# Griffan/FASTQuick

Measured on AMD Instinct MI355X. Metric: paired_150bp_reads_aligned_per_sec, higher is better.
Workload: dtype u32

## Files before the change

fastquick_amd/api.py:

```python
from __future__ import annotations

import ctypes as C
import os

import numpy as np

HERE = os.path.dirname(os.path.abspath(__file__))
DEFAULT_LIB = os.environ.get("FQ_LIB_EXPERIMENT") or os.path.join(HERE, "libfastquick_amd.so")

FQ_K_NAMES = ("prep", "width", "gap", "sa", "sw", "refine", "prep_kernel", "gap_kernel")


class Opts(C.Structure):
    _fields_ = [
        ("s_mm", C.c_int32), ("s_gapo", C.c_int32), ("s_gape", C.c_int32), ("mode", C.c_int32),
        ("indel_end_skip", C.c_int32), ("max_del_occ", C.c_int32), ("max_entries", C.c_int32),
        ("fnr", C.c_double), ("max_diff", C.c_int32), ("max_gapo", C.c_int32), ("max_gape", C.c_int32),
        ("max_seed_diff", C.c_int32), ("seed_len", C.c_int32), ("max_top2", C.c_int32), ("trim_qual", C.c_int32),
        ("filter_thresh", C.c_int32), ("max_isize", C.c_int32), ("force_isize", C.c_int32), ("max_occ", C.c_uint32),
        ("n_multi", C.c_int32), ("N_multi", C.c_int32), ("is_sw", C.c_int32), ("ap_prior", C.c_double),
        ("host_threads", C.c_int32), ("batch_pairs", C.c_int32), ("single_end", C.c_int32), ("pad_opts", C.c_int32),
    ]


# ... 35 lines not shown
class Isize(C.Structure):
    _fields_ = [("avg", C.c_double), ("std", C.c_double), ("ap_prior", C.c_double), ("low", C.c_uint32),
                ("high", C.c_uint32), ("high_bayesian", C.c_uint32), ("pad", C.c_uint32)]


class ResultBatch(C.Structure):
    _fields_ = [("n_pairs", C.c_int32), ("n_survivors", C.c_int32), ("n_both_filtered", C.c_int32),
                ("n_both_unmapped", C.c_int32), ("pair_idx", C.POINTER(C.c_int32)), ("rec", C.POINTER(Result)),
                ("cigar", C.POINTER(C.c_uint16)), ("md", C.c_void_p), ("multi", C.POINTER(Multi)),
                ("isize", Isize), ("n_bases", C.c_int64), ("n_sub", C.c_int32), ("isize_sub", C.POINTER(Isize))]


class Stats(C.Structure):
    _fields_ = [("kernel_ms", C.c_double * 16), ("kernel_launches", C.c_uint64 * 16),
                ("occ_block_touches", C.c_uint64), ("gap_occ_touches", C.c_uint64), ("gap_nogap_touches", C.c_uint64), ("filter_probes", C.c_uint64),
                ("stack_pops", C.c_uint64), ("stack_pushes", C.c_uint64), ("sa_rows", C.c_uint64),
                ("reads_searched", C.c_uint64), ("pairs", C.c_uint64), ("sw_tasks", C.c_uint64),
                ("refine_tasks", C.c_uint64), ("tier_retries", C.c_uint64),
                ("max_pops_per_read", C.c_uint64), ("reads_over_4k_pops", C.c_uint64), ("max_wave_trips", C.c_uint64),
                ("host_ms_serial", C.c_double), ("host_ms_pair", C.c_double), ("host_ms_total", C.c_double),
                ("wall_ms_total", C.c_double), ("wave_trips", C.c_uint64), ("lane_trips", C.c_uint64),
                ("h2d_bytes", C.c_uint64), ("d2h_bytes", C.c_uint64), ("pairs_on_device", C.c_uint64), ("dbg", C.c_uint64 * 16),
                ("width_occ_touches", C.c_uint64), ("md_reads", C.c_uint64), ("host_pairs", C.c_uint64),
                ("device_wait_ms", C.c_double), ("host_cpu_ms", C.c_double), ("dp_launches", C.c_uint64 * 6)]


class FrontEndStats(C.Structure):
    _fields_ = [("ms_inflate", C.c_double), ("ms_tokenise", C.c_double), ("members", C.c_int64), ("refused", C.c_int64),
                ("text_bytes", C.c_int64), ("comp_bytes", C.c_int64), ("pairs", C.c_int64),
                ("ms_lines", C.c_double), ("ms_records", C.c_double), ("ms_slots", C.c_double), ("inflate_launches", C.c_int64), ("chunks", C.c_int64),
                ("ms_wait_reader", C.c_double), ("ms_wait_slot", C.c_double), ("ms_read", C.c_double), ("ms_upload", C.c_double),
                ("bam_records", C.c_int64), ("bam_skipped", C.c_int64), ("chain_repairs", C.c_int64), ("ms_transcode", C.c_double),
                ("ms_bam_starts", C.c_double), ("ms_bam_pairs", C.c_double), ("ms_bam_fill", C.c_double),
                ("bam_orphans", C.c_int64), ("bam_held_peak_records", C.c_int64), ("bam_held_peak_bytes", C.c_int64), ("ms_bam_collate", C.c_double),
                ("bam_unselected", C.c_int64), ("bam_oq_records", C.c_int64), ("ms_bam_tags", C.c_double), ("bam_empty_chunks", C.c_int64)]


class BamCollate(C.Structure):
    _fields_ = [("records", C.c_int64), ("kept", C.c_int64), ("pairs", C.c_int64), ("orphans", C.c_int64), ("held_peak_records", C.c_int64), ("held_peak_bytes", C.c_int64),
                ("text_len", C.c_int64 * 2), ("chain_end", C.c_int64), ("bad_record", C.c_int64),
                ("bad_kind", C.c_int32), ("paired", C.c_int32), ("chunks", C.c_int32), ("end_flag", C.c_int32),
                ("ms_collate", C.c_double), ("ms_keys", C.c_double), ("ms_sort", C.c_double), ("ms_match", C.c_double), ("ms_units", C.c_double), ("ms_hold", C.c_double),
                ("error", C.c_char * 256)]


class BamProbe(C.Structure):
    _fields_ = [("n_ref", C.c_int32), ("paired", C.c_int32), ("first_flag", C.c_int32), ("first_l_seq", C.c_int32), ("first_l_name", C.c_int32), ("has_eof_block", C.c_int32),
# ... 1189 lines not shown
```

fastquick_amd/csrc/fq_align.cpp:

```cpp
#include <algorithm>
#include <atomic>
#include <ctime>
#include <chrono>
#include <climits>
#include <cstdint>
#include <cmath>
#include <cstdio>
#include <cstdlib>
#include <cstring>
#include <memory>
#include <string>
#include <unordered_map>
#include <mutex>
#include <thread>
#include <vector>
#include <pthread.h>
#include <sched.h>

#include "../../include/fastquick_amd.h"
#include "fq_backend.h"
#include "fq_index.h"
#include "fq_pipeline.h"
#include "fq_pool.h"
#include "fq_text_batch.h"
// ... 381 lines not shown
  else if (k == "gap_split_hard") c->kn.gap_split_hard = v;
  else if (k == "gap_long_pops2") c->kn.gap_long_pops2 = (uint32_t)v;
  else if (k == "gap_skip_bound") c->kn.gap_skip_bound = v;
  else if (k == "gap_no_order") c->kn.gap_no_order = (int)v;
  else if (k == "device_turns") c->kn.device_turns = (int)v;
  else if (k == "device_turn_min") c->kn.device_turn_min = v;
  else if (k == "device_turn_slots") c->kn.device_turn_slots = (int)std::max<int64_t>(1, v);
  else if (k == "gap_round2_waves") c->kn.gap_round2_waves = (int)v;
  else if (k == "gap_round2_lane_major") c->kn.gap_round2_lane_major = (int)v;
  else if (k == "gap_round1_refill") c->kn.gap_round1_refill = (int)v;
  else if (k == "gap_round2_refill") c->kn.gap_round2_refill = (int)v;
  else if (k == "sw_wave_max") c->kn.sw_wave_max = (int)v;
  else if (k == "host_threads") c->kn.host_threads = (int)v;
  else if (k == "host_par_min") c->kn.host_par_min = (size_t)v;
  else if (k == "packed_bulk_min") c->kn.packed_bulk_min = v;
  else if (k == "md_mask_min") c->kn.md_mask_min = v;
  else if (k == "trace") c->kn.trace = (int)v;
  else if (k == "gap_order_asc") t->gap_order_asc = (int)v;
  else if (k == "gap_waves_per_cu") t->gap_waves_per_cu = (int)v;
  else if (k == "gap_coop_waves") t->gap_coop_waves = (int)v;
  else if (k == "gap_refill_min") t->gap_refill_min = (int)v;
  else if (k == "filter_no_turns") t->filter_no_turns = (int)v;
  else if (k == "prep_priority") t->prep_priority = (int)v;
  else if (k == "refine_lanes") t->refine_lanes = (int)v;
  else if (k == "gap_generic_opts") t->gap_generic_opts = (int)v;
  else if (k == "sw_serial_reverse") t->sw_serial_reverse = (int)v;
  else if (k == "width_both_strands") t->width_both_strands = (int)v;
  else if (k == "spin_sync") t->spin_sync = (int)v;
  else return FQ_EINVAL;
  return FQ_OK;
}

extern "C" void fq_stats_get(const fq_ctx_t *c, fq_stats_t *out) { if (c && out) *out = c->stats; }
extern "C" void fq_stats_reset(fq_ctx_t *c) { if (c) memset(&c->stats, 0, sizeof c->stats); }

#define CK(expr)                                                  \
  do {                                                            \
    if ((expr)) { c->err = std::string(#expr) + ": " + fqdev::last_error(); return FQ_ENODEV; } \
  } while (0)
#define CKM(expr)                                                 \
  do {                                                            \
    if (!(expr)) { c->err = std::string("out of device memory: ") + #expr; return FQ_ENOMEM; } \
  } while (0)

static int h2d_staged(fq_ctx *c, void *dst, const void *src, size_t bytes) {
  if (!bytes) return 0;
// ... 303 lines not shown
  const fq_text_batch *text = nullptr;
};

int stage0_filter(Call &K, const FilterIn &in) {
  fq_ctx *c = K.c;
  const int n = K.n, n2 = K.n2, n_sub = K.n_sub, B = K.B;
  const bool ascii = !in.head, se = c->o.single_end != 0, ragged = !ascii && in.uniform_len <= 0;
  const int n_in = se ? n : n2;
  const size_t n_max = (size_t)(ascii ? 1 : 3) * n_sub;
  CKM(c->d_filtered.ensure(n2 + 64) && c->d_read_list.ensure(n2) && c->d_sidx.ensure(n2) && c->d_pair_list.ensure(n) && c->d_sub_max.ensure(n_max) && (!ascii || c->d_len_trim.ensure(n2)));
  CK(fqdev::dzero(c->d_sub_max.p, n_max * 4));
  if (se) CK(fqdev::dfill(c->d_filtered.p + n, 1, (size_t)n));
  if (se && ascii) CK(fqdev::dzero(c->d_len_trim.p + n, (size_t)n * 4));
  fqdev::time_begin(FQ_K_PREP);
  if (ascii) {
    FqPrepArgs a{};
    a.ix = c->ix->dev; a.o = c->ko; a.seq = c->d_seq.p; a.qual = c->d_qual.p; a.len = c->d_len.p; a.stride = c->stride; a.n_reads = n_in;
    a.len_trim = c->d_len_trim.p; a.filtered = c->d_filtered.p; a.sub_max = c->d_sub_max.p; a.n_pairs = n; a.batch_pairs = B; a.counters = c->d_counters.p;
    CK(fqdev::launch_prep(a));
  } else {
    FqPrepPackedArgs a{};
    a.ix = c->ix->dev; a.o = c->ko; a.head = in.head; a.len = ragged ? in.len : nullptr; a.uniform_len = in.uniform_len; a.qual_last = in.qual_last; a.sub_whole = c->d_sub_max.p + n_sub;
    a.n_reads = n_in; a.filtered = c->d_filtered.p; a.sub_max = c->d_sub_max.p; a.n_pairs = n; a.batch_pairs = B; a.counters = c->d_counters.p;
    CK(fqdev::launch_prep_packed(a));
  }
  CK(fqdev::launch_compact(c->d_filtered.p, n, c->d_read_list.p, c->d_sidx.p, c->d_pair_list.p, c->d_counts.p));
  fqdev::time_end(FQ_K_PREP);
  int32_t counts[2] = {0, 0};
  c->h_sub_max.assign(n_sub, in.uniform_len);
  K.sub_whole.assign(n_sub, 0);
  std::vector<uint64_t> striped(ragged ? (size_t)FQ_C_STRIPES * FQ_C_STRIDE : 0);
  CKS(d2h_staged(c, counts, c->d_counts.p, 8));
  if (in.qual_last) CKS(d2h_staged(c, K.sub_whole.data(), c->d_sub_max.p + n_sub, (size_t)n_sub * 4));
  if (ascii || ragged) CKS(d2h_staged(c, c->h_sub_max.data(), c->d_sub_max.p, (size_t)n_sub * 4));
  if (ragged) CKS(d2h_staged(c, striped.data(), c->d_counters.p, striped.size() * 8));
  CKS(sync_staged(c));
  K.trace("  stage0: filter + compaction on the device");
  if (ragged) {
    uint64_t folded[FQ_C_COUNT];
    fold_counters(striped.data(), folded);
    if (folded[FQ_C_BADLEN]) return refuse_length(c);
    for (int sb = 0; in.body_stride && sb < n_sub; ++sb)
      if (((int64_t)c->h_sub_max[sb] + 3) / 4 > (int64_t)in.body_stride) { c->err = "a read is longer than body_stride holds"; return FQ_EINVAL; }
    c->n_bases_in = (int64_t)folded[FQ_C_BASES];
  } else if (!ascii) c->n_bases_in = (int64_t)n_in * in.uniform_len;
  K.n_search = counts[0]; K.n_surv = counts[1];
  K.dstride = ascii ? c->stride : (std::max(1, *std::max_element(c->h_sub_max.begin(), c->h_sub_max.end())) + 15) & ~15;
// ... 1780 lines not shown
```

fastquick_amd/csrc/fq_backend.h:

```cpp
#pragma once
#include "fq_kernels.h"
#include "fq_records.h"
#include "fq_frontend.h"
#include "fq_emit.h"
#include "fq_deflate.h"
#include "fq_sort.h"
#include "fq_bamin.h"

namespace fqdev {

struct State;
struct Tune {
  int gap_coop_waves = 0;
  int gap_waves_per_cu = 0, gap_refill_min = 0, gap_order_asc = 0, filter_no_turns = 0, refine_lanes = 0;
  int spin_sync = 0;
  int gap_generic_opts = 0;
  int width_both_strands = 0;
  int prep_priority = 0;
  int sw_serial_reverse = 0;
};
int runtime_configure(int hw_queues, int blocking_waits);
int device_count();
State *state_create(int device_ordinal);
void state_destroy(State *s);
int bind(State *s);
Tune *tune(State *s);
const char *last_error();
bool is_real_gpu();
void device_turn_begin(int slots = 1);
void device_turn_end();

void *dmalloc(size_t bytes);
void dfree(void *p);
void *hmalloc(size_t bytes);
void hfree(void *p);
int h2d(void *dst, const void *src, size_t bytes);
int d2h(void *dst, const void *src, size_t bytes);
int copy_pinned(void *dst, const void *src, size_t bytes, int to_device);
int d2d(void *dst, const void *src, size_t bytes);
int dzero(void *dst, size_t bytes);
int dfill(void *dst, int byte, size_t bytes);
int sync();
int h2d_copy(void *dst, const void *src, size_t bytes);
int copy_record(int slot);
int copy_wait(int slot);
void copy_discard();
int compute_wait_copy(int slot);
int copy_flush_now();

void time_begin(int kid);
void time_end(int kid);
void time_collect(double ms[], uint64_t launches[], int n_ids);
inline thread_local uint64_t dp_launches[FQ_DP_COUNT] = {};

int launch_prep(const FqPrepArgs &a);
int launch_compact(const uint8_t *filtered, int n_pairs, int32_t *read_list, int32_t *sidx, int32_t *pair_list, int32_t *counts);
int launch_surv_gather(const int32_t *pair_list, int n_surv, int n_pairs, const int32_t *len_trim, const uint8_t *filtered, const int32_t *sidx, FqSurvInfo *out);
int launch_prep_packed(const FqPrepPackedArgs &a);
int launch_surv_map(const int32_t *pair_list, int n_surv, int n_pairs, const uint8_t *filtered, const int32_t *sidx, FqSurvInfo *out,
                    int32_t *row_map, int32_t *read_list_c, int32_t *crow_of);
int launch_unpack(const FqUnpackArgs &a);
int launch_patch(const FqPatchArgs &a);
int launch_trim(const FqTrimArgs &a);
int launch_trim_all(const FqTrimAllArgs &a);
int launch_width(const FqWidthArgs &a);
int launch_order(const uint8_t *bid_end, int n, int n_hard, int32_t *order, uint32_t *cnt);
int gap_lane_slots(const FqGapArgs &a);
int launch_gap(const FqGapArgs &a);
int launch_scan(const uint32_t *in, uint64_t *out, uint32_t n);
int launch_pack_aln(const FqAln *aln, const uint32_t *n_aln, const uint64_t *off, uint32_t cap, uint32_t n_work, FqAln *packed);
int launch_sa(const FqSaArgs &a);
int stream_aux(int on);
int stream_fork();
int stream_join();
int stream_mark(int k);
int stream_wait_mark(int k);
// ... 27 lines not shown
```

fastquick_amd/csrc/fq_device.hip:

```cpp
#include <hip/hip_runtime.h>
#include <hip/hip_ext.h>

#include <algorithm>
#include <condition_variable>
#include <atomic>
#include <cstdio>
#include <cstdlib>
#include <cstring>
#include <mutex>
#include <string>
#include <unordered_map>
#include <vector>
#include <sys/mman.h>
#include <sys/syscall.h>
#include <unistd.h>

#include "fq_backend.h"
#define FQ_PC_KERNELS
#include "fq_popcon.h"
#define FQ_SVD_KERNELS
#include "fq_svd.h"
#define FQ_VCF_KERNELS
#include "fq_vcf.h"

// ... 33 lines not shown
      return -3;                                                                             \
    }                                                                                        \
  } while (0)

int copy_flush();
#define FQ_PRE() do { if (copy_flush()) return -3; } while (0)
void copy_discard() { if (g_cur) g_cur->n_small = 0; }
int copy_flush_now() { FQ_PRE(); return 0; }

const char *last_error() { return g_err.c_str(); }
bool is_real_gpu() { return true; }

static int set_kernel_attributes();
static std::mutex g_dev_mu;
static bool g_dev_ready[64];
static hipEvent_t g_prep_last[64];
static State *g_prep_owner[64];
static hipStream_t g_copy_streams[64][2];
static unsigned g_copy_next[64];
static std::mutex g_turn_mu[64];
static std::condition_variable g_turn_cv[64];
static int g_turn_held[64];
static int g_ctx_count[64];
static hipStream_t g_prio_stream[64];
static bool g_queue_warned = false;
static int g_rt_blocking_waits = 0;
int runtime_configure(int hw_queues, int blocking_waits) {
  if (hw_queues > 0) {
    char b[16];
    snprintf(b, sizeof b, "%d", hw_queues);
    setenv("GPU_MAX_HW_QUEUES", b, 0);
  }
  g_rt_blocking_waits = blocking_waits ? 1 : 0;
  return 0;
}

int device_count() { int n = 0; if (hipGetDeviceCount(&n) != hipSuccess) { (void)hipGetLastError(); return 0; } return n < 0 ? 0 : n; }
void device_turn_begin(int slots) {
  const int d = g_cur->device;
  std::unique_lock<std::mutex> lk(g_turn_mu[d]);
  g_turn_cv[d].wait(lk, [&] { return g_turn_held[d] < (slots < 1 ? 1 : slots); });
  ++g_turn_held[d];
}
void device_turn_end() {
  const int d = g_cur->device;
  { std::lock_guard<std::mutex> lk(g_turn_mu[d]); --g_turn_held[d]; }
// ... 28 lines not shown
            hipEventCreateWithFlags(&s->copy_done[1], hipEventDisableTiming | hipEventBlockingSync) == hipSuccess &&
            hipEventCreateWithFlags(&s->prep_done, hipEventDisableTiming) == hipSuccess &&
            hipEventCreateWithFlags(&s->sync_ev, hipEventDisableTiming | hipEventBlockingSync) == hipSuccess;
  if (!ok) { g_err = "stream / event creation failed"; state_destroy(s); return nullptr; }
  s->main_stream = s->stream;
  return s;
}
void state_destroy(State *s) {
  if (!s) return;
  (void)hipSetDevice(s->device);
  g_cur = nullptr;
  s->stream = s->main_stream ? s->main_stream : s->stream;
  if (s->aux_stream) { (void)hipStreamSynchronize(s->aux_stream); (void)hipStreamDestroy(s->aux_stream); }
  if (s->sync_ev) (void)hipEventDestroy(s->sync_ev);
  if (s->fork_ev) (void)hipEventDestroy(s->fork_ev);
  if (s->join_ev) (void)hipEventDestroy(s->join_ev);
  for (hipEvent_t m : s->marks) if (m) (void)hipEventDestroy(m);
  if (s->prio_fork) (void)hipEventDestroy(s->prio_fork);
  if (s->stream) (void)hipStreamSynchronize(s->stream);
  if (s->copy_stream) (void)hipStreamSynchronize(s->copy_stream);
  {
    std::lock_guard<std::mutex> lk(g_dev_mu);
    if (g_prep_owner[s->device] == s) { g_prep_owner[s->device] = nullptr; g_prep_last[s->device] = nullptr; }
    if (g_ctx_count[s->device] > 0) --g_ctx_count[s->device];
  }
  for (auto &p : s->pending) { (void)hipEventDestroy(p.a); (void)hipEventDestroy(p.b); }
  for (auto e : s->free_events) (void)hipEventDestroy(e);
  for (auto e : s->copy_done) if (e) (void)hipEventDestroy(e);
  if (s->prep_done) (void)hipEventDestroy(s->prep_done);
  if (s->scan_tmp) (void)hipFree(s->scan_tmp);
  if (s->cmp_cnt) (void)hipFree(s->cmp_cnt);
  if (s->cmp_off) (void)hipFree(s->cmp_off);
  if (s->stream) (void)hipStreamDestroy(s->stream);
  delete s;
}
Tune *tune(State *s) { return &s->tune; }
int bind(State *s) {
  if (!s) { g_err = "no device state"; return -3; }
  if (g_cur != s) { FQ_HIP(hipSetDevice(s->device)); g_cur = s; }
  return 0;
}

void *dmalloc(size_t bytes) {
  void *p = nullptr;
  if (hipMalloc(&p, bytes ? bytes : 16) != hipSuccess) { g_err = "hipMalloc failed (" + std::to_string(bytes) + " B)"; return nullptr; }
  return p;
}
// ... 889 lines not shown
    FQ_HIP(hipEventRecord(g_cur->prep_done, g_stream));
    g_prep_last[dev] = g_cur->prep_done; g_prep_owner[dev] = g_cur;
  } else {
    hipExtLaunchKernelGGL(k_prep, dim3(nblk((uint64_t)a.n_reads, 256)), dim3(256), 0, g_stream, e0, e1, 0, a);
  }
  FQ_HIP(hipGetLastError());
  return 0;
}
__global__ void __launch_bounds__(256) k_surv_gather(const int32_t *pair_list, int n_surv, int n_pairs, const int32_t *len_trim, const uint8_t *filtered, const int32_t *sidx, FqSurvInfo *out) {
  const int t = blockIdx.x * blockDim.x + threadIdx.x;
  if (t < 2 * n_surv) fq_surv_gather_thread(pair_list, n_pairs, len_trim, filtered, sidx, out, t);
}
int launch_surv_gather(const int32_t *pair_list, int n_surv, int n_pairs, const int32_t *len_trim, const uint8_t *filtered, const int32_t *sidx, FqSurvInfo *out) {
  FQ_PRE();
  if (n_surv <= 0) return 0;
  hipLaunchKernelGGL(k_surv_gather, dim3(nblk((uint64_t)n_surv * 2, 256)), dim3(256), 0, g_stream, pair_list, n_surv, n_pairs, len_trim, filtered, sidx, out);
  FQ_HIP(hipGetLastError());
  return 0;
}
__global__ void __launch_bounds__(256) k_prep_packed(FqPrepPackedArgs a) {
  const int r = blockIdx.x * blockDim.x + threadIdx.x;
  if (r < a.n_reads) fq_prep_packed_thread(a, r);
}
int launch_prep_packed(const FqPrepPackedArgs &a) {
  FQ_PRE();
  if (a.n_reads <= 0) return 0;
  hipEvent_t e0, e1;
  kernel_events(FQ_K_PREP_KERNEL, &e0, &e1);
  const dim3 grid(nblk((uint64_t)a.n_reads, 256));
  hipStream_t st = g_stream;
  if (g_cur->tune.prep_priority) {
    {
      std::lock_guard<std::mutex> lk(g_dev_mu);
      if (!g_prio_stream[g_cur->device]) {
        int lo = 0, hi = 0;
        FQ_HIP(hipDeviceGetStreamPriorityRange(&lo, &hi));
        FQ_HIP(hipStreamCreateWithPriority(&g_prio_stream[g_cur->device], hipStreamNonBlocking, hi));
      }
    }
    if (!g_cur->prio_fork) FQ_HIP(hipEventCreateWithFlags(&g_cur->prio_fork, hipEventDisableTiming));
    FQ_HIP(hipEventRecord(g_cur->prio_fork, g_stream));
    FQ_HIP(hipStreamWaitEvent(g_prio_stream[g_cur->device], g_cur->prio_fork, 0));
    st = g_prio_stream[g_cur->device];
  }
  if (!g_cur->tune.filter_no_turns) {
    const int dev = g_cur->device;
    std::lock_guard<std::mutex> lk(g_dev_mu);
    if (g_prep_last[dev] && g_prep_owner[dev] != g_cur) FQ_HIP(hipStreamWaitEvent(st, g_prep_last[dev], 0));
    hipExtLaunchKernelGGL(k_prep_packed, grid, dim3(256), 0, st, e0, e1, 0, a);
    FQ_HIP(hipEventRecord(g_cur->prep_done, st));
    g_prep_last[dev] = g_cur->prep_done; g_prep_owner[dev] = g_cur;
    if (st != g_stream) FQ_HIP(hipStreamWaitEvent(g_stream, g_cur->prep_done, 0));
  } else {
    hipExtLaunchKernelGGL(k_prep_packed, grid, dim3(256), 0, st, e0, e1, 0, a);
    if (st != g_stream) { FQ_HIP(hipEventRecord(g_cur->prep_done, st)); FQ_HIP(hipStreamWaitEvent(g_stream, g_cur->prep_done, 0)); }
  }
  FQ_HIP(hipGetLastError());
  return 0;
}
__global__ void __launch_bounds__(256) k_surv_map(const int32_t *pair_list, int n_surv, int n_pairs, const uint8_t *filtered, const int32_t *sidx, FqSurvInfo *out,
                                                  int32_t *row_map, int32_t *read_list_c, int32_t *crow_of) {
  const int t = blockIdx.x * blockDim.x + threadIdx.x;
  if (t < 2 * n_surv) fq_surv_map_thread(pair_list, n_pairs, filtered, sidx, out, row_map, read_list_c, crow_of, t);
}
int launch_surv_map(const int32_t *pair_list, int n_surv, int n_pairs, const uint8_t *filtered, const int32_t *sidx, FqSurvInfo *out,
                    int32_t *row_map, int32_t *read_list_c, int32_t *crow_of) {
  FQ_PRE();
  if (n_surv <= 0) return 0;
  hipLaunchKernelGGL(k_surv_map, dim3(nblk((uint64_t)n_surv * 2, 256)), dim3(256), 0, g_stream, pair_list, n_surv, n_pairs, filtered, sidx, out, row_map, read_list_c, crow_of);
  FQ_HIP(hipGetLastError());
  return 0;
}
// ... 939 lines not shown
```

fastquick_amd/csrc/fq_kernels.h:

```cpp
#pragma once
#include "fq_common.h"

#define FQ_LAMBDA_INLINE __attribute__((always_inline))
#if defined(__HIP_DEVICE_COMPILE__)
#define FQ_POPC64(x) __popcll(x)
#define FQ_POPC32(x) __popc(x)
#define FQ_CTZ32(x) (__ffs((int)(x)) - 1)
#define FQ_C_STRIPE_OFF ((size_t)(blockIdx.x & (FQ_C_STRIPES - 1)) * FQ_C_STRIDE)
#define FQ_ATOMIC_ADD64(p, v) atomicAdd((unsigned long long *)(p) + FQ_C_STRIPE_OFF, (unsigned long long)(v))
#define FQ_ATOMIC_MAX64(p, v) atomicMax((unsigned long long *)(p) + FQ_C_STRIPE_OFF, (unsigned long long)(v))
#define FQ_LOAD_RELAXED(p) __hip_atomic_load((p), __ATOMIC_RELAXED, __HIP_MEMORY_SCOPE_AGENT)
#define FQ_ATOMIC_MAX32(p, v) do { const int fq_v_ = (int)(v); if (fq_v_ > FQ_LOAD_RELAXED((const int *)(p))) atomicMax((int *)(p), fq_v_); } while (0)
#define FQ_WAVE_COUNT(p, pred)                                                                                      \
  do {                                                                                                              \
    const unsigned long long m_ = __ballot((pred) ? 1 : 0);                                                         \
    if ((pred) && __lane_id() == (unsigned)(__ffsll((long long)m_) - 1)) atomicAdd((unsigned long long *)(p) + FQ_C_STRIPE_OFF, (unsigned long long)__popcll(m_)); \
  } while (0)
#else
#define FQ_WAVE_COUNT(p, pred) do { if (pred) *(p) += 1; } while (0)
#define FQ_LOAD_RELAXED(p) (*(p))
#define FQ_ATOMIC_MAX32(p, v) (*(p) = *(p) > (int32_t)(v) ? *(p) : (int32_t)(v))
#define FQ_ATOMIC_MAX64(p, v) (*(p) = *(p) > (uint64_t)(v) ? *(p) : (uint64_t)(v))
#define FQ_POPC64(x) __builtin_popcountll(x)
#define FQ_POPC32(x) __builtin_popcount(x)
// ... 296 lines not shown
    uint64_t km = d;
    if (var) {
      const int sh = 2 * (int)(i - half);
      const uint64_t a = (A.alleles[lo] >> (2 * v)) & 3u;
      km = (km & ~((uint64_t)3 << sh)) | (a << sh);
    }
    for (int t = 0; t < 6; ++t) set_bit(t, fq_kmer_project(km, t));
  }
}

struct FqPrepPackedArgs {
  FqDevIndex ix;
  FqKOpts o;
  const uint64_t *head;
  const uint16_t *len;
  int32_t uniform_len;
  int32_t n_reads;
  uint8_t *filtered;
  int32_t *sub_max;
  const uint8_t *qual_last;
  int32_t *sub_whole;
  int32_t n_pairs, batch_pairs;
  uint64_t *counters;
};
FQ_HD void fq_prep_packed_thread(const FqPrepPackedArgs &A, int r) {
  if (A.qual_last) {
    const int len = A.len ? (int)A.len[r] : A.uniform_len;
    const int qsub = (A.o.mode & FQ_MODE_IL13) ? 31 : 0;
    const bool whole = len - 1 < 34 || A.o.trim_qual - ((int)(uint8_t)(A.qual_last[r] - qsub) - 33) < 0;
    const int slot = (r >= A.n_pairs ? r - A.n_pairs : r) / A.batch_pairs;
#if defined(__HIP_DEVICE_COMPILE__)
    int mx = whole ? len : 0;
    const int slot0 = __builtin_amdgcn_readfirstlane(slot);
    if (__ballot(slot != slot0) == 0) {
#pragma unroll
      for (int d = 32; d >= 1; d >>= 1) { const int o = __shfl_xor(mx, d); mx = o > mx ? o : mx; }
      if (mx > 0 && __lane_id() == (unsigned)(__ffsll((long long)__ballot(1)) - 1)) FQ_ATOMIC_MAX32(&A.sub_whole[slot0], mx);
    } else if (mx > 0) FQ_ATOMIC_MAX32(&A.sub_whole[slot], mx);
#else
    if (whole && A.sub_whole[slot] < len) A.sub_whole[slot] = len;
#endif
  }
  if (A.len) {
    const int len = A.len[r];
    const int slot = (r >= A.n_pairs ? r - A.n_pairs : r) / A.batch_pairs;
    FQ_ATOMIC_MAX32(&A.sub_max[slot], len);
    FQ_ATOMIC_ADD64(&A.counters[FQ_C_BASES], (uint64_t)len);
    if (len < FQ_LMIN || len > FQ_LMAX) FQ_ATOMIC_ADD64(&A.counters[FQ_C_BADLEN], 1);
  }
  uint8_t filt = 0;
  if (A.o.filter_thresh != 0) {
    uint64_t kmer[3];
#pragma unroll
    for (int ch = 0; ch < 3; ++ch) kmer[ch] = A.head[(size_t)ch * (size_t)A.n_reads + (size_t)r];
    const int th = A.o.filter_thresh;
    uint8_t byte[18];
    uint32_t bit[18], off[18];
#pragma unroll
    for (int ch = 0; ch < 3; ++ch)
#pragma unroll
      for (int t = 0; t < 6; ++t) {
        const uint32_t x = fq_kmer_project(kmer[ch], t);
        off[6 * ch + t] = x >> 3;
        bit[6 * ch + t] = x & 7u;
      }
#pragma unroll
    for (int q = 0; q < 16; ++q) byte[q] = A.ix.bitmap[q % 6][off[q]];
    byte[16] = byte[17] = 0;
    if (th < 3) { byte[16] = A.ix.bitmap[4][off[16]]; byte[17] = A.ix.bitmap[5][off[17]]; }
    int c16 = 0;
#pragma unroll
    for (int q = 0; q < 16; ++q) c16 += (byte[q] >> bit[q]) & 1;
    if (th >= 3 && c16 + 2 >= th) { byte[16] = A.ix.bitmap[4][off[16]]; byte[17] = A.ix.bitmap[5][off[17]]; }
    int cnt[3] = {0, 0, 0};
#pragma unroll
    for (int ch = 0; ch < 3; ++ch)
#pragma unroll
      for (int t = 0; t < 6; ++t) cnt[ch] += (byte[6 * ch + t] >> bit[6 * ch + t]) & 1;
    const bool p0 = cnt[0] >= th, p1 = cnt[0] + cnt[1] >= th, p2 = cnt[0] + cnt[1] + cnt[2] >= th;
    filt = p2 ? 0 : 1;
    const uint32_t probes = p0 ? 6u : p1 ? 12u : 18u;
#if defined(__HIP_DEVICE_COMPILE__)
    uint32_t ps = probes;
#pragma unroll
    for (int d = 32; d >= 1; d >>= 1) ps += (uint32_t)__shfl_xor((int)ps, d);
    if (__lane_id() == (unsigned)(__ffsll((long long)__ballot(1)) - 1)) FQ_ATOMIC_ADD64(&A.counters[FQ_C_PROBES], ps);
#else
    FQ_ATOMIC_ADD64(&A.counters[FQ_C_PROBES], probes);
#endif
  }
  A.filtered[r] = filt;
}

struct FqUnpackArgs {
  const uint8_t *body;
  int32_t body_stride;
  const int32_t *row_map;
  const uint16_t *len;
  int32_t uniform_len;
  int32_t n_rows;
  uint8_t *seq;
  int32_t stride;
  int32_t *len_out;
  int32_t *len_trim;
};
FQ_HD void fq_unpack_piece(const FqUnpackArgs &A, int64_t g) {
  const int per_row = A.stride >> 4;
  const int t = (int)(g / per_row), cidx = (int)(g - (int64_t)t * per_row);
  const size_t src = A.row_map ? (size_t)A.row_map[t] : (size_t)t;
  const int len = A.len ? (int)A.len[src] : A.uniform_len;
  const uint8_t *b = A.body + src * (size_t)A.body_stride + 4 * (size_t)cidx;
  const int p0 = 16 * cidx;
  uint32_t v = 0;
#pragma unroll
// ... 1950 lines not shown
```

include/fastquick_amd.h:

```cpp
#ifndef FASTQUICK_AMD_H
#define FASTQUICK_AMD_H
#include <stddef.h>
#include <stdint.h>

#ifdef __cplusplus
extern "C" {
#endif

#define FQ_OK 0
#define FQ_EINVAL (-1)
#define FQ_EIO (-2)
#define FQ_ENODEV (-3)
#define FQ_ENOMEM (-4)
#define FQ_ELIMIT (-5)

#define FQ_TYPE_NO_MATCH 0
#define FQ_TYPE_UNIQUE 1
#define FQ_TYPE_REPEAT 2
#define FQ_TYPE_MATESW 3
#define FQ_MAX_READ_LEN 500

typedef struct fq_index fq_index_t;
typedef struct fq_ctx fq_ctx_t;

// ... 336 lines not shown
  uint64_t kernel_launches[FQ_K_COUNT];
  uint64_t occ_block_touches;
  uint64_t gap_occ_touches;
  uint64_t gap_nogap_touches;
  uint64_t filter_probes;
  uint64_t stack_pops, stack_pushes;
  uint64_t sa_rows;
  uint64_t reads_searched, pairs, sw_tasks, refine_tasks;
  uint64_t tier_retries;
  uint64_t max_pops_per_read, reads_over_4k_pops;
  uint64_t max_wave_trips;
  double host_ms_serial, host_ms_pair, host_ms_total, wall_ms_total;
  uint64_t wave_trips;
  uint64_t lane_trips;
  uint64_t h2d_bytes, d2h_bytes;
  uint64_t pairs_on_device;
  uint64_t dbg[16];
  uint64_t width_occ_touches;
  uint64_t md_reads;
  uint64_t host_pairs;
  double device_wait_ms;
  double host_cpu_ms;
  uint64_t dp_launches[FQ_DP_COUNT];
} fq_stats_t;
void fq_stats_get(const fq_ctx_t *c, fq_stats_t *out);
void fq_stats_reset(fq_ctx_t *c);

const char *fq_version(void);
int fq_host_cpus(void);
int fq_runtime_configure(int hw_queues, int blocking_waits);
int fq_device_count(void);
int fq_index_bitmap_fetch(const fq_index_t *ix, int32_t t, uint8_t *out);

typedef struct fq_popcon fq_popcon_t;
typedef struct {
  int32_t num_pc;
  int32_t within_ancestry;
  int32_t disable_sanity_check;
  int32_t fix_pc;
  int32_t fix_alpha;
  int32_t host_eval;
  int32_t device;
  int32_t host_threads;
  double fix_pc_values[8];
  double fix_alpha_value;
  double epsilon;
// ... 76 lines not shown
```

Baseline: 758.0 million.

## Bin k-mer filter probes by bitmap region before probing

For large packed batches, the read prefilter no longer probes the six bitmap tables with scattered per-read loads. It now counts, bucket-sorts and scatters every k-mer probe by table and high key byte into per-region lists, probes each 2MB region in XCD-grouped chunks, ORs the hit bits into a per-read mask, and computes the verdict in a final pass. The aim is to turn random DRAM/cache misses into region-local accesses with better L2 locality. In exchange it adds five launches, device scratch buffers, atomics, and always probes the first 16 (or 18) k-mers instead of reading the last two lazily. It only applies above a batch-size threshold.

Result: faster. 924.0 million (median of 6 runs) (+21.9%).

```diff
diff --git a/fastquick_amd/api.py b/fastquick_amd/api.py
--- a/fastquick_amd/api.py
+++ b/fastquick_amd/api.py
@@ -81,7 +81,8 @@
                 ("wall_ms_total", C.c_double), ("wave_trips", C.c_uint64), ("lane_trips", C.c_uint64),
                 ("h2d_bytes", C.c_uint64), ("d2h_bytes", C.c_uint64), ("pairs_on_device", C.c_uint64), ("dbg", C.c_uint64 * 16),
                 ("width_occ_touches", C.c_uint64), ("md_reads", C.c_uint64), ("host_pairs", C.c_uint64),
-                ("device_wait_ms", C.c_double), ("host_cpu_ms", C.c_double), ("dp_launches", C.c_uint64 * 6)]
+                ("device_wait_ms", C.c_double), ("host_cpu_ms", C.c_double), ("dp_launches", C.c_uint64 * 6),
+                ("filter_binned_reads", C.c_uint64), ("filter_bin_spill", C.c_uint64)]
 
 
 class FrontEndStats(C.Structure):
diff --git a/fastquick_amd/csrc/fq_align.cpp b/fastquick_amd/csrc/fq_align.cpp
--- a/fastquick_amd/csrc/fq_align.cpp
+++ b/fastquick_amd/csrc/fq_align.cpp
@@ -427,6 +427,7 @@
   else if (k == "gap_refill_min") t->gap_refill_min = (int)v;
   else if (k == "filter_no_turns") t->filter_no_turns = (int)v;
   else if (k == "prep_priority") t->prep_priority = (int)v;
+  else if (k == "filter_binned_min") t->filter_binned_min = std::max<int64_t>(0, v);
   else if (k == "refine_lanes") t->refine_lanes = (int)v;
   else if (k == "gap_generic_opts") t->gap_generic_opts = (int)v;
   else if (k == "sw_serial_reverse") t->sw_serial_reverse = (int)v;
@@ -776,7 +777,12 @@
     FqPrepPackedArgs a{};
     a.ix = c->ix->dev; a.o = c->ko; a.head = in.head; a.len = ragged ? in.len : nullptr; a.uniform_len = in.uniform_len; a.qual_last = in.qual_last; a.sub_whole = c->d_sub_max.p + n_sub;
     a.n_reads = n_in; a.filtered = c->d_filtered.p; a.sub_max = c->d_sub_max.p; a.n_pairs = n; a.batch_pairs = B; a.counters = c->d_counters.p;
-    CK(fqdev::launch_prep_packed(a));
+    const fqdev::Tune *tn = fqdev::tune(c->dev);
+    a.binned = c->ko.filter_thresh != 0 && !tn->filter_no_turns && (int64_t)n_in >= tn->filter_binned_min && n_in < FQ_BIN_MAX_READS;
+    const int rc = fqdev::launch_prep_packed(a);
+    c->stats.filter_binned_reads += fqdev::filter_binned_reads; c->stats.filter_bin_spill += fqdev::filter_bin_spill;
+    fqdev::filter_binned_reads = fqdev::filter_bin_spill = 0;
+    CK(rc);
   }
   CK(fqdev::launch_compact(c->d_filtered.p, n, c->d_read_list.p, c->d_sidx.p, c->d_pair_list.p, c->d_counts.p));
   fqdev::time_end(FQ_K_PREP);
diff --git a/fastquick_amd/csrc/fq_backend.h b/fastquick_amd/csrc/fq_backend.h
--- a/fastquick_amd/csrc/fq_backend.h
+++ b/fastquick_amd/csrc/fq_backend.h
@@ -17,6 +17,7 @@
   int gap_generic_opts = 0;
   int width_both_strands = 0;
   int prep_priority = 0;
+  int64_t filter_binned_min = 2621440;
   int sw_serial_reverse = 0;
 };
 int runtime_configure(int hw_queues, int blocking_waits);
@@ -52,6 +53,7 @@
 void time_end(int kid);
 void time_collect(double ms[], uint64_t launches[], int n_ids);
 inline thread_local uint64_t dp_launches[FQ_DP_COUNT] = {};
+inline thread_local uint64_t filter_binned_reads = 0, filter_bin_spill = 0;
 
 int launch_prep(const FqPrepArgs &a);
 int launch_compact(const uint8_t *filtered, int n_pairs, int32_t *read_list, int32_t *sidx, int32_t *pair_list, int32_t *counts);
diff --git a/fastquick_amd/csrc/fq_device.hip b/fastquick_amd/csrc/fq_device.hip
--- a/fastquick_amd/csrc/fq_device.hip
+++ b/fastquick_amd/csrc/fq_device.hip
@@ -79,6 +79,7 @@
 static std::condition_variable g_turn_cv[64];
 static int g_turn_held[64];
 static int g_ctx_count[64];
+static void bin_scratch_free(int dev);
 static hipStream_t g_prio_stream[64];
 static bool g_queue_warned = false;
 static int g_rt_blocking_waits = 0;
@@ -153,7 +154,7 @@
   {
     std::lock_guard<std::mutex> lk(g_dev_mu);
     if (g_prep_owner[s->device] == s) { g_prep_owner[s->device] = nullptr; g_prep_last[s->device] = nullptr; }
-    if (g_ctx_count[s->device] > 0) --g_ctx_count[s->device];
+    if (g_ctx_count[s->device] > 0 && --g_ctx_count[s->device] == 0) bin_scratch_free(s->device);
   }
   for (auto &p : s->pending) { (void)hipEventDestroy(p.a); (void)hipEventDestroy(p.b); }
   for (auto e : s->free_events) (void)hipEventDestroy(e);
@@ -1089,12 +1090,183 @@
   const int r = blockIdx.x * blockDim.x + threadIdx.x;
   if (r < a.n_reads) fq_prep_packed_thread(a, r);
 }
+struct BinScratch {
+  FqBinEntry *ent = nullptr; size_t ent_cap = 0;
+  uint32_t *mask = nullptr; size_t mask_cap = 0;
+  uint32_t *count = nullptr, *base = nullptr, *cursor = nullptr, *chunks = nullptr;
+  std::vector<void *> retired;
+};
+static BinScratch g_bin[64];
+static void bin_scratch_free(int dev) {
+  BinScratch &b = g_bin[dev];
+  for (void *p : b.retired) (void)hipFree(p);
+  if (b.ent) (void)hipFree(b.ent);
+  if (b.mask) (void)hipFree(b.mask);
+  if (b.count) (void)hipFree(b.count);
+  b = BinScratch();
+}
+static int bin_scratch_ensure(int dev, size_t n_ent, size_t n_reads, hipStream_t st) {
+  BinScratch &b = g_bin[dev];
+  if (!b.count) {
+    constexpr size_t n = 4 * (size_t)FQ_BIN_BUCKETS + 2;
+    FQ_HIP(hipMalloc((void **)&b.count, n * 4));
+    b.base = b.count + FQ_BIN_BUCKETS; b.cursor = b.base + FQ_BIN_BUCKETS + 1; b.chunks = b.cursor + FQ_BIN_BUCKETS;
+    FQ_HIP(hipMemsetAsync(b.count, 0, n * 4, st));
+  }
+  if (n_ent > b.ent_cap) {
+    if (b.ent) b.retired.push_back(b.ent);
+    b.ent = nullptr; b.ent_cap = 0;
+    const size_t want = n_ent + n_ent / 8;
+    FQ_HIP(hipMalloc((void **)&b.ent, want * sizeof(FqBinEntry)));
+    b.ent_cap = want;
+  }
+  if (n_reads > b.mask_cap) {
+    if (b.mask) b.retired.push_back(b.mask);
+    b.mask = nullptr; b.mask_cap = 0;
+    const size_t want = n_reads + n_reads / 8;
+    FQ_HIP(hipMalloc((void **)&b.mask, want * 4));
+    b.mask_cap = want;
+    FQ_HIP(hipMemsetAsync(b.mask, 0, want * 4, st));
+  }
+  return 0;
+}
+constexpr int kBinThreads = 1024, kBinTile = 2 * kBinThreads;
+constexpr int kBinProbeThreads = 512, kBinProbePer = 2, kBinChunk = kBinProbeThreads * kBinProbePer;
+constexpr int kBinProbeWgPerXcd = 32;
+__device__ inline void bin_kmers(const FqPrepPackedArgs &a, int r, uint64_t kmer[3]) {
+#pragma unroll
+  for (int ch = 0; ch < 3; ++ch) kmer[ch] = a.head[(size_t)ch * (size_t)a.n_reads + (size_t)r];
+}
+__global__ void __launch_bounds__(kBinThreads) k_prep_bin_count(FqPrepPackedArgs a, uint32_t *__restrict__ count) {
+  __shared__ uint32_t h[FQ_BIN_BUCKETS];
+  for (int i = threadIdx.x; i < FQ_BIN_BUCKETS; i += kBinThreads) h[i] = 0;
+  __syncthreads();
+  const int front = fq_filter_front(a.o.filter_thresh);
+  for (int64_t r = (int64_t)blockIdx.x * kBinThreads + threadIdx.x; r < a.n_reads; r += (int64_t)gridDim.x * kBinThreads) {
+    uint64_t kmer[3];
+    bin_kmers(a, (int)r, kmer);
+#pragma unroll
+    for (int q = 0; q < 18; ++q) if (q < front) atomicAdd(&h[fq_bin_pos(q, fq_filter_key(kmer, q))], 1u);
+  }
+  __syncthreads();
+  for (int i = threadIdx.x; i < FQ_BIN_BUCKETS; i += kBinThreads) if (h[i]) atomicAdd(&count[i], h[i]);
+}
+__global__ void __launch_bounds__(256) k_prep_bin_offsets(uint32_t *__restrict__ count, uint32_t *__restrict__ base, uint32_t *__restrict__ cursor, uint32_t *__restrict__ chunks) {
+  static_assert(FQ_BIN_BUCKETS == 6 * 256, "six buckets per thread");
+  __shared__ uint32_t se[256], sc[256];
+  const int t = threadIdx.x;
+  uint32_t c[6], e = 0, k = 0;
+  for (int j = 0; j < 6; ++j) { c[j] = count[6 * t + j]; count[6 * t + j] = 0; e += c[j]; k += (c[j] + kBinChunk - 1) / kBinChunk; }
+  se[t] = e; sc[t] = k;
+  __syncthreads();
+  for (int d = 1; d < 256; d <<= 1) {
+    const uint32_t ae = t >= d ? se[t - d] : 0, ac = t >= d ? sc[t - d] : 0;
+    __syncthreads();
+    se[t] += ae; sc[t] += ac;
+    __syncthreads();
+  }
+  e = se[t] - e; k = sc[t] - k;
+  for (int j = 0; j < 6; ++j) { base[6 * t + j] = e; cursor[6 * t + j] = e; chunks[6 * t + j] = k; e += c[j]; k += (c[j] + kBinChunk - 1) / kBinChunk; }
+  if (t == 255) { base[FQ_BIN_BUCKETS] = e; chunks[FQ_BIN_BUCKETS] = k; }
+}
+__global__ void __launch_bounds__(kBinThreads) k_prep_bin(FqPrepPackedArgs a, FqBinEntry *__restrict__ ent, uint32_t *__restrict__ cursor) {
+  constexpr int RPT = kBinTile / kBinThreads;
+  __shared__ FqBinEntry sorted[kBinTile * 3];
+  __shared__ uint32_t h[256], start[256], delta[256];
+  const int tid = threadIdx.x, front = fq_filter_front(a.o.filter_thresh);
+  const int n_tiles = (a.n_reads + kBinTile - 1) / kBinTile;
+  for (int tile = blockIdx.x; tile < n_tiles; tile += gridDim.x) {
+    uint64_t kmer[RPT][3];
+#pragma unroll
+    for (int i = 0; i < RPT; ++i) {
+      const int64_t r = (int64_t)tile * kBinTile + i * kBinThreads + tid;
+      if (r < a.n_reads) bin_kmers(a, (int)r, kmer[i]);
+    }
+    for (int t = 0; t < 6; ++t) {
+      if (tid < 256) h[tid] = 0;
+      __syncthreads();
+      uint32_t key[RPT][3], rank[RPT][3];
+#pragma unroll
+      for (int i = 0; i < RPT; ++i) {
+        const int64_t r = (int64_t)tile * kBinTile + i * kBinThreads + tid;
+#pragma unroll
+        for (int j = 0; j < 3; ++j)
+          if (t + 6 * j < front && r < a.n_reads) { key[i][j] = fq_kmer_project(kmer[i][j], t); rank[i][j] = atomicAdd(&h[key[i][j] >> 24], 1u); }
+      }
+      __syncthreads();
+      if (tid < 256) start[tid] = h[tid];
+      __syncthreads();
+      for (int d = 1; d < 256; d <<= 1) {
+        const uint32_t add = (tid < 256 && tid >= d) ? start[tid - d] : 0;
+        __syncthreads();
+        if (tid < 256) start[tid] += add;
+        __syncthreads();
+      }
+      const uint32_t n_ent = start[255];
+      __syncthreads();
+      if (tid < 256) {
+        const uint32_t c = h[tid], s = start[tid] - c;
+        start[tid] = s;
+        if (c) delta[tid] = atomicAdd(&cursor[fq_bin_pos(t, (uint32_t)tid << 24)], c) - s;
+      }
+      __syncthreads();
+#pragma unroll
+      for (int i = 0; i < RPT; ++i) {
+        const int64_t r = (int64_t)tile * kBinTile + i * kBinThreads + tid;
+#pragma unroll
+        for (int j = 0; j < 3; ++j)
+          if (t + 6 * j < front && r < a.n_reads) sorted[start[key[i][j] >> 24] + rank[i][j]] = fq_bin_entry(key[i][j], (int)r, t + 6 * j);
+      }
+      __syncthreads();
+      for (uint32_t i = tid; i < n_ent; i += kBinThreads) { const FqBinEntry e = sorted[i]; ent[delta[e.key >> 24] + i] = e; }
+      __syncthreads();
+    }
+  }
+}
+__global__ void __launch_bounds__(kBinProbeThreads) k_prep_bin_probe(FqDevIndex ix, const FqBinEntry *__restrict__ ent, const uint32_t *__restrict__ base,
+                                                                     const uint32_t *__restrict__ chunks, uint32_t *__restrict__ mask) {
+  const int x = blockIdx.x % FQ_BIN_XCDS;
+  const uint32_t per = gridDim.x / FQ_BIN_XCDS, c0 = chunks[x * FQ_BIN_PER_XCD], c1 = chunks[(x + 1) * FQ_BIN_PER_XCD];
+  for (uint32_t k = c0 + blockIdx.x / FQ_BIN_XCDS; k < c1; k += per) {
+    int lo = x * FQ_BIN_PER_XCD, hi = (x + 1) * FQ_BIN_PER_XCD;
+    while (hi - lo > 1) { const int mid = (lo + hi) >> 1; if (chunks[mid] <= k) lo = mid; else hi = mid; }
+    const uint8_t *region = fq_bin_region(ix, lo);
+    const uint32_t first = base[lo] + (k - chunks[lo]) * kBinChunk, end = base[lo + 1];
+    FqBinEntry e[kBinProbePer]; uint32_t hit[kBinProbePer];
+#pragma unroll
+    for (int i = 0; i < kBinProbePer; ++i) {
+      const uint32_t at = first + i * kBinProbeThreads + threadIdx.x;
+      if (at < end) e[i] = ent[at]; else e[i].tag = ~0u;
+    }
+#pragma unroll
+    for (int i = 0; i < kBinProbePer; ++i) hit[i] = e[i].tag != ~0u ? fq_bin_hit(region, e[i]) : 0;
+#pragma unroll
+    for (int i = 0; i < kBinProbePer; ++i) if (hit[i]) atomicOr(&mask[fq_bin_read(e[i])], fq_bin_mask_bit(e[i]));
+  }
+}
+__global__ void __launch_bounds__(256) k_prep_bin_verdict(FqPrepPackedArgs a, uint32_t *__restrict__ mask) {
+  const int r = blockIdx.x * blockDim.x + threadIdx.x;
+  if (r < a.n_reads) fq_prep_binned_verdict_thread(a, mask, r);
+}
+static int launch_prep_binned(const FqPrepPackedArgs &a, hipStream_t st, hipEvent_t e0, hipEvent_t e1) {
+  const BinScratch &b = g_bin[g_cur->device];
+  FQ_HIP(hipEventRecord(e0, st));
+  hipLaunchKernelGGL(k_prep_bin_count, dim3(std::min<unsigned>(512, nblk((uint64_t)a.n_reads, kBinThreads))), dim3(kBinThreads), 0, st, a, b.count);
+  hipLaunchKernelGGL(k_prep_bin_offsets, dim3(1), dim3(256), 0, st, b.count, b.base, b.cursor, b.chunks);
+  hipLaunchKernelGGL(k_prep_bin, dim3(std::min<unsigned>(512, nblk((uint64_t)a.n_reads, kBinTile))), dim3(kBinThreads), 0, st, a, b.ent, b.cursor);
+  hipLaunchKernelGGL(k_prep_bin_probe, dim3(FQ_BIN_XCDS * kBinProbeWgPerXcd), dim3(kBinProbeThreads), 0, st, a.ix, (const FqBinEntry *)b.ent, (const uint32_t *)b.base, (const uint32_t *)b.chunks, b.mask);
+  hipLaunchKernelGGL(k_prep_bin_verdict, dim3(nblk((uint64_t)a.n_reads, 256)), dim3(256), 0, st, a, b.mask);
+  FQ_HIP(hipEventRecord(e1, st));
+  filter_binned_reads += (uint64_t)a.n_reads;
+  return 0;
+}
 int launch_prep_packed(const FqPrepPackedArgs &a) {
   FQ_PRE();
   if (a.n_reads <= 0) return 0;
   hipEvent_t e0, e1;
   kernel_events(FQ_K_PREP_KERNEL, &e0, &e1);
   const dim3 grid(nblk((uint64_t)a.n_reads, 256));
+  bool binned = a.binned && a.o.filter_thresh != 0 && !g_cur->tune.filter_no_turns && a.n_reads < FQ_BIN_MAX_READS;
   hipStream_t st = g_stream;
   if (g_cur->tune.prep_priority) {
     {
@@ -1113,8 +1285,10 @@
   if (!g_cur->tune.filter_no_turns) {
     const int dev = g_cur->device;
     std::lock_guard<std::mutex> lk(g_dev_mu);
-    if (g_prep_last[dev] && g_prep_owner[dev] != g_cur) FQ_HIP(hipStreamWaitEvent(st, g_prep_last[dev], 0));
-    hipExtLaunchKernelGGL(k_prep_packed, grid, dim3(256), 0, st, e0, e1, 0, a);
+    if (binned && bin_scratch_ensure(dev, (size_t)a.n_reads * (size_t)fq_filter_front(a.o.filter_thresh), (size_t)a.n_reads, st)) { (void)hipGetLastError(); binned = false; }
+    if (g_prep_last[dev] && (g_prep_owner[dev] != g_cur || binned)) FQ_HIP(hipStreamWaitEvent(st, g_prep_last[dev], 0));
+    if (binned) { if (launch_prep_binned(a, st, e0, e1)) return -3; }
+    else hipExtLaunchKernelGGL(k_prep_packed, grid, dim3(256), 0, st, e0, e1, 0, a);
     FQ_HIP(hipEventRecord(g_cur->prep_done, st));
     g_prep_last[dev] = g_cur->prep_done; g_prep_owner[dev] = g_cur;
     if (st != g_stream) FQ_HIP(hipStreamWaitEvent(g_stream, g_cur->prep_done, 0));
diff --git a/fastquick_amd/csrc/fq_kernels.h b/fastquick_amd/csrc/fq_kernels.h
--- a/fastquick_amd/csrc/fq_kernels.h
+++ b/fastquick_amd/csrc/fq_kernels.h
@@ -342,8 +342,9 @@
   int32_t *sub_whole;
   int32_t n_pairs, batch_pairs;
   uint64_t *counters;
+  int32_t binned;
 };
-FQ_HD void fq_prep_packed_thread(const FqPrepPackedArgs &A, int r) {
+FQ_HD void fq_prep_packed_lengths(const FqPrepPackedArgs &A, int r) {
   if (A.qual_last) {
     const int len = A.len ? (int)A.len[r] : A.uniform_len;
     const int qsub = (A.o.mode & FQ_MODE_IL13) ? 31 : 0;
@@ -368,48 +369,71 @@
     FQ_ATOMIC_ADD64(&A.counters[FQ_C_BASES], (uint64_t)len);
     if (len < FQ_LMIN || len > FQ_LMAX) FQ_ATOMIC_ADD64(&A.counters[FQ_C_BADLEN], 1);
   }
+}
+FQ_HD int fq_filter_front(int thresh) { return thresh >= 3 ? 16 : 18; }
+FQ_HD uint32_t fq_filter_key(const uint64_t kmer[3], int q) { return fq_kmer_project(kmer[q / 6], q % 6); }
+FQ_HD uint8_t fq_prep_packed_verdict(const FqPrepPackedArgs &A, const uint64_t kmer[3], uint32_t hits) {
+  const int th = A.o.filter_thresh;
+  if (th >= 3 && FQ_POPC32(hits & 0xffffu) + 2 >= th)
+    for (int q = 16; q < 18; ++q) { const uint32_t x = fq_filter_key(kmer, q); hits |= (uint32_t)((A.ix.bitmap[q % 6][x >> 3] >> (x & 7u)) & 1u) << q; }
+  int cnt[3];
+#pragma unroll
+  for (int ch = 0; ch < 3; ++ch) cnt[ch] = FQ_POPC32((hits >> (6 * ch)) & 63u);
+  const bool p0 = cnt[0] >= th, p1 = cnt[0] + cnt[1] >= th, p2 = cnt[0] + cnt[1] + cnt[2] >= th;
+  const uint32_t probes = p0 ? 6u : p1 ? 12u : 18u;
+#if defined(__HIP_DEVICE_COMPILE__)
+  uint32_t ps = probes;
+#pragma unroll
+  for (int d = 32; d >= 1; d >>= 1) ps += (uint32_t)__shfl_xor((int)ps, d);
+  if (__lane_id() == (unsigned)(__ffsll((long long)__ballot(1)) - 1)) FQ_ATOMIC_ADD64(&A.counters[FQ_C_PROBES], ps);
+#else
+  FQ_ATOMIC_ADD64(&A.counters[FQ_C_PROBES], probes);
+#endif
+  return p2 ? 0 : 1;
+}
+FQ_HD void fq_prep_packed_thread(const FqPrepPackedArgs &A, int r) {
+  fq_prep_packed_lengths(A, r);
   uint8_t filt = 0;
   if (A.o.filter_thresh != 0) {
     uint64_t kmer[3];
 #pragma unroll
     for (int ch = 0; ch < 3; ++ch) kmer[ch] = A.head[(size_t)ch * (size_t)A.n_reads + (size_t)r];
-    const int th = A.o.filter_thresh;
     uint8_t byte[18];
     uint32_t bit[18], off[18];
 #pragma unroll
-    for (int ch = 0; ch < 3; ++ch)
-#pragma unroll
-      for (int t = 0; t < 6; ++t) {
-        const uint32_t x = fq_kmer_project(kmer[ch], t);
-        off[6 * ch + t] = x >> 3;
-        bit[6 * ch + t] = x & 7u;
-      }
+    for (int q = 0; q < 18; ++q) { const uint32_t x = fq_filter_key(kmer, q); off[q] = x >> 3; bit[q] = x & 7u; }
 #pragma unroll
     for (int q = 0; q < 16; ++q) byte[q] = A.ix.bitmap[q % 6][off[q]];
     byte[16] = byte[17] = 0;
-    if (th < 3) { byte[16] = A.ix.bitmap[4][off[16]]; byte[17] = A.ix.bitmap[5][off[17]]; }
-    int c16 = 0;
-#pragma unroll
-    for (int q = 0; q < 16; ++q) c16 += (byte[q] >> bit[q]) & 1;
-    if (th >= 3 && c16 + 2 >= th) { byte[16] = A.ix.bitmap[4][off[16]]; byte[17] = A.ix.bitmap[5][off[17]]; }
-    int cnt[3] = {0, 0, 0};
-#pragma unroll
-    for (int ch = 0; ch < 3; ++ch)
-#pragma unroll
-      for (int t = 0; t < 6; ++t) cnt[ch] += (byte[6 * ch + t] >> bit[6 * ch + t]) & 1;
-    const bool p0 = cnt[0] >= th, p1 = cnt[0] + cnt[1] >= th, p2 = cnt[0] + cnt[1] + cnt[2] >= th;
-    filt = p2 ? 0 : 1;
-    const uint32_t probes = p0 ? 6u : p1 ? 12u : 18u;
-#if defined(__HIP_DEVICE_COMPILE__)
-    uint32_t ps = probes;
-#pragma unroll
-    for (int d = 32; d >= 1; d >>= 1) ps += (uint32_t)__shfl_xor((int)ps, d);
-    if (__lane_id() == (unsigned)(__ffsll((long long)__ballot(1)) - 1)) FQ_ATOMIC_ADD64(&A.counters[FQ_C_PROBES], ps);
-#else
-    FQ_ATOMIC_ADD64(&A.counters[FQ_C_PROBES], probes);
-#endif
+    if (fq_filter_front(A.o.filter_thresh) == 18) { byte[16] = A.ix.bitmap[4][off[16]]; byte[17] = A.ix.bitmap[5][off[17]]; }
+    uint32_t hits = 0;
+#pragma unroll
+    for (int q = 0; q < 18; ++q) hits |= (uint32_t)((byte[q] >> bit[q]) & 1u) << q;
+    filt = fq_prep_packed_verdict(A, kmer, hits);
   }
   A.filtered[r] = filt;
+}
+
+constexpr int FQ_BIN_BUCKETS = 6 * 256, FQ_BIN_XCDS = 8, FQ_BIN_PER_XCD = FQ_BIN_BUCKETS / FQ_BIN_XCDS;
+constexpr int FQ_BIN_MAX_READS = 1 << 27;
+struct FqBinEntry { uint32_t key, tag; };
+FQ_HD int fq_bin_pos(int q, uint32_t key) { const int b = (q % 6) * 256 + (int)(key >> 24); return (b % FQ_BIN_XCDS) * FQ_BIN_PER_XCD + b / FQ_BIN_XCDS; }
+FQ_HD FqBinEntry fq_bin_entry(uint32_t key, int r, int q) { FqBinEntry e; e.key = key; e.tag = (uint32_t)r << 5 | (uint32_t)q; return e; }
+FQ_HD const uint8_t *fq_bin_region(const FqDevIndex &ix, int p) {
+  const int b = (p % FQ_BIN_PER_XCD) * FQ_BIN_XCDS + p / FQ_BIN_PER_XCD;
+  return ix.bitmap[b >> 8] + ((size_t)(b & 255) << 21);
+}
+FQ_HD uint32_t fq_bin_hit(const uint8_t *region, FqBinEntry e) { return (uint32_t)((region[(e.key & 0xffffffu) >> 3] >> (e.key & 7u)) & 1u); }
+FQ_HD int fq_bin_read(FqBinEntry e) { return (int)(e.tag >> 5); }
+FQ_HD uint32_t fq_bin_mask_bit(FqBinEntry e) { return 1u << (e.tag & 31u); }
+FQ_HD void fq_prep_binned_verdict_thread(const FqPrepPackedArgs &A, uint32_t *mask, int r) {
+  fq_prep_packed_lengths(A, r);
+  uint64_t kmer[3];
+#pragma unroll
+  for (int ch = 0; ch < 3; ++ch) kmer[ch] = A.head[(size_t)ch * (size_t)A.n_reads + (size_t)r];
+  const uint32_t hits = mask[r];
+  if (hits) mask[r] = 0;
+  A.filtered[r] = fq_prep_packed_verdict(A, kmer, hits);
 }
 
 struct FqUnpackArgs {
diff --git a/include/fastquick_amd.h b/include/fastquick_amd.h
--- a/include/fastquick_amd.h
+++ b/include/fastquick_amd.h
@@ -382,6 +382,8 @@
   double device_wait_ms;
   double host_cpu_ms;
   uint64_t dp_launches[FQ_DP_COUNT];
+  uint64_t filter_binned_reads;
+  uint64_t filter_bin_spill;
 } fq_stats_t;
 void fq_stats_get(const fq_ctx_t *c, fq_stats_t *out);
 void fq_stats_reset(fq_ctx_t *c);
```
